# Xinran1205/LBM-Asynchronous

Measured on AMD Instinct MI355X. Metric: MLUPS, higher is better.
Workload: dtype f32

## Files before the change

### include/lbm_hip.h

```cpp
#ifndef LBM_HIP_H
#define LBM_HIP_H

#include <stddef.h>

#ifdef __cplusplus
extern "C" {
#endif

#define LBM_SUCCESS 0
#define LBM_FAILURE 1

#define LBM_ERRORS_DIE    0
#define LBM_ERRORS_RETURN 1

#define LBM_MATH_EXACT 0
#define LBM_MATH_FAST  1

#define LBM_HALO_SYNC  0
#define LBM_HALO_STALE 1
#define LBM_HALO_FRESHEST 2

typedef struct {
  int   nx;
  int   ny;
  int   max_iters;
  int   reynolds_dim;
  float density;
  float accel;
  float omega;
} lbm_params;

typedef struct lbm_ctx lbm_ctx;

typedef struct {
  int    n_slabs;
  int    row_first;
  int    row_count;
  int    fluid_cells;
  int    steps_done;
  int    math_mode;
  int    world_rank;
  int    world_size;
  int    steps_per_launch;
  int    halo_mode;
  int    band_rows;
  int    lane_cells;
  int    nontemporal;
  int    graph_steps;
  int    resident_steps;
  int    resident_min_steps;
  int    resident_rows;
  int    resident_group;
  int    resident_one_xcd;
} lbm_info;

void        lbm_set_error_mode(int mode);
const char* lbm_last_error(void);

const char* lbm_version(void);
int         lbm_device_count(void);

int lbm_partition_rows(int ny, int parts, int index, int* first, int* count);

typedef struct {
  int is_send;
  int peer;
  int row_first;
  int row_count;
} lbm_halo_op;
int lbm_halo_plan(int rows, int parts, int index, int depth, lbm_halo_op out[4]);
int lbm_plan_halo_depth(const lbm_params* params, int parts, int math_mode);

lbm_ctx* lbm_create(const lbm_params* params, const int* obstacles, const float* cells_aos,
                    int n_gpus, int math_mode);

#define LBM_RCCL_ID_BYTES 128
int      lbm_rccl_unique_id(void* id_out);

typedef struct {
  int  loaded;
  int  version;
  int  n_comms;
  int  nranks;
  int  rank;
  char library[512];
} lbm_rccl_status;
// ... 75 lines not shown
```

### lbm-asynchronous_amd/__init__.py

```python
from __future__ import annotations

import ctypes
import os
import subprocess
from dataclasses import dataclass

import numpy as np

_HERE = os.path.dirname(os.path.abspath(__file__))
LIB_PATH = os.environ.get("LBM_LIB") or os.path.join(_HERE, "liblbm_hip.so")
CLI_PATH = os.path.join(_HERE, "d2q9-bgk")

MATH_EXACT = 0
MATH_FAST = 1
_MATH = {"exact": MATH_EXACT, "fast": MATH_FAST, MATH_EXACT: MATH_EXACT, MATH_FAST: MATH_FAST}
RCCL_ID_BYTES = 128
MASK_HALO_ROWS = 3
HALO_SYNC = 0
HALO_STALE = 1
HALO_FRESHEST = 2
_HALO = {"sync": HALO_SYNC, "stale": HALO_STALE, "freshest": HALO_FRESHEST,
         HALO_SYNC: HALO_SYNC, HALO_STALE: HALO_STALE, HALO_FRESHEST: HALO_FRESHEST}

ABI_SYMBOLS = (
    "lbm_set_error_mode", "lbm_last_error", "lbm_version", "lbm_device_count",
    "lbm_partition_rows", "lbm_halo_plan", "lbm_plan_halo_depth", "lbm_create", "lbm_rccl_unique_id", "lbm_rccl_info", "lbm_create_rank", "lbm_create_rank_rows",
    "lbm_create_tiled", "lbm_create_rank_tiled", "lbm_create_rank_hosted", "lbm_create_rank_hosted_rows",
    "lbm_create_rank_hosted_tiled", "lbm_destroy",
    "lbm_get_info", "lbm_set_halo_mode", "lbm_read_halo_log", "lbm_run", "lbm_sync", "lbm_run_timed", "lbm_read_av_vels", "lbm_read_cells",
    "lbm_read_final_state", "lbm_av_velocity", "lbm_total_density", "lbm_calc_reynolds",
    "lbm_set_frames", "lbm_read_frames",
    "lbm_create_batch", "lbm_batch_member", "lbm_batch_run", "lbm_batch_sync", "lbm_batch_get_info", "lbm_destroy_batch",
)


class LbmError(RuntimeError):
    pass


class _CParams(ctypes.Structure):
    _fields_ = [("nx", ctypes.c_int), ("ny", ctypes.c_int), ("max_iters", ctypes.c_int),
                ("reynolds_dim", ctypes.c_int), ("density", ctypes.c_float),
                ("accel", ctypes.c_float), ("omega", ctypes.c_float)]


class _CInfo(ctypes.Structure):
    _fields_ = [("n_slabs", ctypes.c_int), ("row_first", ctypes.c_int), ("row_count", ctypes.c_int),
                ("fluid_cells", ctypes.c_int), ("steps_done", ctypes.c_int),
                ("math_mode", ctypes.c_int), ("world_rank", ctypes.c_int),
                ("world_size", ctypes.c_int), ("steps_per_launch", ctypes.c_int),
                ("halo_mode", ctypes.c_int), ("band_rows", ctypes.c_int), ("lane_cells", ctypes.c_int),
                ("nontemporal", ctypes.c_int), ("graph_steps", ctypes.c_int),
                ("resident_steps", ctypes.c_int), ("resident_min_steps", ctypes.c_int),
                ("resident_rows", ctypes.c_int), ("resident_group", ctypes.c_int), ("resident_one_xcd", ctypes.c_int)]


class _CBatchInfo(ctypes.Structure):
    _fields_ = [("members", ctypes.c_int), ("members_per_launch", ctypes.c_int), ("launches_per_chunk", ctypes.c_int),
                ("resident_steps", ctypes.c_int), ("resident_min_steps", ctypes.c_int), ("steps_done", ctypes.c_int)]


class _CRcclStatus(ctypes.Structure):
    _fields_ = [("loaded", ctypes.c_int), ("version", ctypes.c_int), ("n_comms", ctypes.c_int),
                ("nranks", ctypes.c_int), ("rank", ctypes.c_int), ("library", ctypes.c_char * 512)]


class _CHaloOp(ctypes.Structure):
    _fields_ = [("is_send", ctypes.c_int), ("peer", ctypes.c_int), ("row_first", ctypes.c_int),
                ("row_count", ctypes.c_int)]


_EXCHANGE_FN = ctypes.CFUNCTYPE(ctypes.c_int, ctypes.c_void_p, ctypes.c_int, ctypes.POINTER(_CHaloOp),
                                ctypes.POINTER(ctypes.POINTER(ctypes.c_float)), ctypes.c_size_t)
_ALLREDUCE_FN = ctypes.CFUNCTYPE(ctypes.c_int, ctypes.c_void_p, ctypes.POINTER(ctypes.c_double), ctypes.c_int)


class _CHostComm(ctypes.Structure):
    _fields_ = [("exchange", _EXCHANGE_FN), ("allreduce_sum", _ALLREDUCE_FN), ("user", ctypes.c_void_p)]


@dataclass
class Params:
    nx: int
    ny: int
    max_iters: int
    reynolds_dim: int
    density: float
# ... 530 lines not shown
```

### lbm-asynchronous_amd/csrc/lbm_hip.hip

```cpp
#include "../../include/lbm_hip.h"
#include "lbm_kernels.hip.h"

#include <hip/hip_runtime.h>
#include <hip/hip_ext.h>
#include <rccl/rccl.h>

#include <dlfcn.h>
#include <algorithm>

#include <atomic>
#include <condition_variable>
#include <cstdarg>
#include <cstdio>
#include <cstdlib>
#include <cstring>
#include <functional>
#include <mutex>
#include <thread>
#include <vector>

namespace {

constexpr int kMaxSlabs = 8;
constexpr int kPartSlots = lbm::kPartSlotsMax;
// ... 78 lines not shown
  }
  bool ok = true;
  auto sym = [&](const char* name) -> void* {
    void* p = dlsym(r.handle, name);
    if (!p) { ok = false; snprintf(g_rccl_error, sizeof(g_rccl_error), "librccl lacks %s", name); }
    return p;
  };
#define LBM_RCCL_SYM(field, name) r.field = reinterpret_cast<decltype(r.field)>(sym(name))
  LBM_RCCL_SYM(GetVersion, "ncclGetVersion");        LBM_RCCL_SYM(GetUniqueId, "ncclGetUniqueId");
  LBM_RCCL_SYM(CommInitRank, "ncclCommInitRank");    LBM_RCCL_SYM(CommInitAll, "ncclCommInitAll");
  LBM_RCCL_SYM(CommDestroy, "ncclCommDestroy");      LBM_RCCL_SYM(CommCount, "ncclCommCount");
  LBM_RCCL_SYM(CommUserRank, "ncclCommUserRank");    LBM_RCCL_SYM(GroupStart, "ncclGroupStart");
  LBM_RCCL_SYM(GroupEnd, "ncclGroupEnd");            LBM_RCCL_SYM(Send, "ncclSend");
  LBM_RCCL_SYM(Recv, "ncclRecv");                    LBM_RCCL_SYM(AllReduce, "ncclAllReduce");
  LBM_RCCL_SYM(GetErrorString, "ncclGetErrorString");
#undef LBM_RCCL_SYM
  if (!ok) { r.handle = nullptr; return; }
  Dl_info di;
  if (dladdr(reinterpret_cast<void*>(r.GetVersion), &di) && di.dli_fname) {
    char real[512];
    const char* shown = realpath(di.dli_fname, real) ? real : di.dli_fname;
    strncpy(r.path, shown, sizeof(r.path) - 1);
  }
}

RcclApi* rccl() {
  std::call_once(g_rccl_once, rccl_bind);
  return g_rccl.handle ? &g_rccl : nullptr;
}

#define RCCL_OR_FAIL(ret)                                                       \
  RcclApi* rc_api_ = rccl();                                                    \
  if (!rc_api_) LBM_FAIL(ret, "RCCL is not available: %s", g_rccl_error)

struct Slab {
  int device = 0;
  int row_first = 0;
  int rows = 0;
  int accel_row = lbm::kNoRow;
  int accel_row2 = lbm::kNoRow;
  float* lat_alloc[2] = {nullptr, nullptr};
  float* lat[2] = {nullptr, nullptr};
  unsigned char* mask_alloc = nullptr;
  unsigned char* mask = nullptr;
  float* partials = nullptr;
  double* tot_u = nullptr;
  double* scratch = nullptr;
  double* reduce_buf = nullptr;
  int* flushed_dev = nullptr;
  uint4* res_gran = nullptr;
  float* res_part = nullptr;
  int* res_status = nullptr;
  int* res_status_host = nullptr;
  float* frames = nullptr;
  hipGraphExec_t chunk_graph[2] = {nullptr, nullptr};
  hipStream_t compute = nullptr, comm = nullptr;
  hipEvent_t ev_boundary = nullptr, ev_halo = nullptr, ev_t0 = nullptr, ev_t1 = nullptr;
  hipEvent_t ev_interior[2] = {nullptr, nullptr};
  hipEvent_t ev_flush = nullptr;
  hipEvent_t ev_step = nullptr;
  hipEvent_t ev_fork = nullptr;
  hipEvent_t ev_x[2] = {nullptr, nullptr};
  float* fresh_stage = nullptr;
  unsigned* fresh_arrived = nullptr;
  unsigned* fresh_id_src = nullptr;
  int* fresh_decision = nullptr;
  unsigned char* fresh_log = nullptr;
  hipEvent_t ev_fresh[2] = {nullptr, nullptr};
  ncclComm_t nccl = nullptr;
  lbm::SlotCounts slot_counts;
  int blocks_main = 0;
  int blocks_boundary = 0;
  long fluid_cells = 0;
};

constexpr int kSumBlocks = 1024;
constexpr int kResidentChunk = 4096;
struct TileShape { int tw, th, kmax, threads; void (*exact)(const lbm::TileArgs); void (*fast)(const lbm::TileArgs); };
#define LBM_TILE_SHAPE(TW, TH, K, T) {TW, TH, K, T, lbm::step_tile<0, TW, TH, K, T>, lbm::step_tile<1, TW, TH, K, T>}
const TileShape kTileShapes[] = {
    LBM_TILE_SHAPE(16, 8, 4, 384),
    LBM_TILE_SHAPE(16, 8, 8, 768),
    LBM_TILE_SHAPE(32, 16, 2, 640),
    LBM_TILE_SHAPE(32, 16, 3, 768),
    LBM_TILE_SHAPE(32, 16, 4, 896),
    LBM_TILE_SHAPE(64, 16, 2, 640),
    LBM_TILE_SHAPE(64, 8, 2, 704),
};
constexpr int kTileShapeCount = (int)(sizeof(kTileShapes) / sizeof(kTileShapes[0]));
constexpr int kHaloRows = 4;
constexpr int kMaskHalo = LBM_MASK_HALO_ROWS;
static_assert(kMaskHalo == kHaloRows - 1, "mask halo");

enum ObstacleKind { OBST_GLOBAL = 0, OBST_ROWS = 1, OBST_TILE = 2 };
struct ObstacleSource {
// ... 95 lines not shown
  long plane_stride = 0;
  long row_pitch = 0;
  int n_slabs = 0;
  Slab slab[kMaxSlabs];
  int cur = 0;
  int steps_done = 0;
  int capacity = 0;
  int fluid_cells = 0;
  int math_mode = LBM_MATH_EXACT;
  int halo = HALO_SELF;
  int halo_mode = LBM_HALO_SYNC;
  int rank = 0, world = 1;
  bool ranked = false;
  bool hosted = false;
  lbm_host_comm host_comm = {nullptr, nullptr, nullptr};
  float* host_send[2] = {nullptr, nullptr};
  float* host_recv[2] = {nullptr, nullptr};
  int row_first = 0, row_count = 0;
  int slot_fill = 0;
  long part_stride = 0;
  bool vec4 = false;
  int neigh = 0;
  int nts = 1;
  int snake = 0;
  int fuse2 = 0;
  int pass_steps = 2;
  int prefetch = 0;
  int xcd_chunk = 0;
  int use_stepk = 0;
  int packed = 0;
  int halo_lanes = 1;
  int lds_windows = 0;
  int band_rows = 8, n_strips = 0;
  int lane_cells = 4;
  SlabTeam* team = nullptr;
  int use_graph = 0;
  GraphBuilder* builder = nullptr;
  int resident = 0;
  int resident_min_steps = 16;
  int resident_bands = 0;
  int resident_joint = 0;
  int resident_rows = 4;
  int resident_group = 1;
  int resident_one_xcd = 0;
  long long resident_timeout = 0;
  bool resident_used = false;
  int tile_steps = 0;
  int tile_shape = 0;
  lbm_batch* batch = nullptr;
  int frame_every = 0;
  int frame_slots = 0;
  int frame_ord0 = 0;
  long long frames_written = 0;
  long long frames_read = 0;
};

struct lbm_batch {
  std::vector<lbm_ctx*> members;
  hipStream_t stream = nullptr;
  int resident = 0;
  int member_wgs = 0;
  int members_per_launch = 1;
  int launches = 0;
  int cur = 0;
  int steps_done = 0;
  lbm::ResidentMember* table = nullptr;
// ... 443 lines not shown
        return LBM_SUCCESS;
      }) != LBM_SUCCESS)
    return LBM_FAILURE;
  if (halo &&
      for_slabs(c, [&](int s) -> int {
        Slab& sl = c->slab[s];
        HIP_TRY(LBM_FAILURE, hipSetDevice(sl.device));
        if (q_wait(c, sl.comm, sl.ev_interior[(m + 1) & 1]) != LBM_SUCCESS) return LBM_FAILURE;
        if (c->halo == HALO_MEMCPY) {
          const int north = (s + 1) % c->n_slabs, south = (s - 1 + c->n_slabs) % c->n_slabs;
          if (q_wait(c, sl.comm, c->slab[north].ev_halo) != LBM_SUCCESS) return LBM_FAILURE;
          if (q_wait(c, sl.comm, c->slab[south].ev_halo) != LBM_SUCCESS) return LBM_FAILURE;
        }
        hipEvent_t bdone = bound_events ? sl.ev_boundary : nullptr;
        if (k) {
          const int off = c->n_strips * ceil_div(sl.rows - 2 * k, c->band_rows);
          if (launch_pass(c, s, sl.comm, k, 0, sl.rows, k, sl.rows - k, 2, off, accel_after, bdone) != LBM_SUCCESS) return LBM_FAILURE;
        } else {
          if (launch_step(c, s, sl.comm, 0, sl.rows - 1, 2, sl.blocks_main, accel_after, bdone) != LBM_SUCCESS) return LBM_FAILURE;
        }
        if (!bdone) return q_record(c, sl.ev_boundary, sl.comm);
        return LBM_SUCCESS;
      }) != LBM_SUCCESS)
    return LBM_FAILURE;
  for (int s = 0; s < c->n_slabs; s++) {
    Slab& sl = c->slab[s];
    const int fused_waves = halo ? c->n_strips * (ceil_div(sl.rows - 2 * k, c->band_rows) + 2)
                                 : c->n_strips * ceil_div(sl.rows, c->band_rows);
    const int n_part = tile ? tile_count(c) : (k ? fused_waves : sl.blocks_main + sl.blocks_boundary);
    for (int j = 0; j < adv; j++) sl.slot_counts.n[c->slot_fill + j] = n_part;
  }
  c->cur ^= 1;
  c->slot_fill += adv;
  return LBM_SUCCESS;
}

int chunk_passes(const lbm_ctx* c, int* steps_per_pass) {
  const int halo = (c->halo != HALO_SELF);
  const int adv = (!halo && c->tile_steps) ? c->tile_steps : (c->fuse2 ? c->pass_steps : 1);
  int passes = kPartSlots / adv;
  const int cap = env_int("LBM_GRAPH_PASSES", 0);
  if (cap > 0 && passes > cap) passes = cap;
  passes -= passes & 1;
  *steps_per_pass = adv;
  return passes;
}

bool graph_is_sound(hipGraph_t graph, const char* dump_path) {
  size_t n_nodes = 0, n_edges = 0;
  if (hipGraphGetNodes(graph, nullptr, &n_nodes) != hipSuccess || hipGraphGetEdges(graph, nullptr, nullptr, &n_edges) != hipSuccess)
    return true;
  if (dump_path) fprintf(stderr, "lbm_hip graph: %zu nodes, %zu edges reported\n", n_nodes, n_edges);
  std::vector<hipGraphNode_t> nodes(n_nodes), from(n_edges), to(n_edges);
  if (n_nodes && hipGraphGetNodes(graph, nodes.data(), &n_nodes) != hipSuccess) return true;
  if (n_edges && hipGraphGetEdges(graph, from.data(), to.data(), &n_edges) != hipSuccess) return true;
  auto index_of = [&](hipGraphNode_t x) -> long {
    for (size_t i = 0; i < n_nodes; i++) if (nodes[i] == x) return (long)i;
    return -1;
  };
  std::vector<long> a(n_edges), b(n_edges);
  std::vector<int> indeg(n_nodes, 0);
  size_t self_edges = 0, dup_edges = 0, foreign = 0;
  for (size_t e = 0; e < n_edges; e++) {
    a[e] = index_of(from[e]);
    b[e] = index_of(to[e]);
    if (a[e] < 0 || b[e] < 0) { foreign++; continue; }
// ... 324 lines not shown
                             sl.lat[c->cur], sl.mask, c->plane_stride, c->row_pitch, c->pitch, c->p.nx,
                             sl.accel_row, a1, a2);
          HIP_TRY(LBM_FAILURE, hipGetLastError());
        }
        if (record_t0) HIP_TRY(LBM_FAILURE, hipEventRecord(sl.ev_t0, sl.compute));
        return LBM_SUCCESS;
      }) != LBM_SUCCESS)
    return LBM_FAILURE;

  if (resident) {
    const long long frames = frames_between(c, c->steps_done, (long long)c->steps_done + n_steps);
    if (run_resident(c, n_steps) != LBM_SUCCESS) return LBM_FAILURE;
    c->steps_done += n_steps;
    c->frames_written += frames;
    return LBM_SUCCESS;
  }

  int flushed_upto = c->steps_done;
  int t_first = 0;
  if (c->use_graph) {
    if (replay_chunks(c, n_steps, flushed_upto, &t_first) != LBM_SUCCESS) return LBM_FAILURE;
    flushed_upto += t_first;
  }
  if (halo && reset_pipeline(c) != LBM_SUCCESS) return LBM_FAILURE;

  static const int ext_events = env_int("LBM_EXT_EVENTS", 1);
  const int slots_per_pass = c->tile_steps > c->pass_steps ? c->tile_steps : c->pass_steps;
  int m = 0;
  for (int t = t_first; t < n_steps; m++) {
    const int tile = (!halo && c->tile_steps) ? (c->tile_steps < n_steps - t ? c->tile_steps : n_steps - t) : 0;
    const int k = (!tile && c->fuse2 && n_steps - t >= 2) ? (n_steps - t >= c->pass_steps ? c->pass_steps : 2) : 0;
    const int adv = tile ? tile : (k ? k : 1);
    const bool last = (t + adv == n_steps);
    if (issue_pass(c, m, tile, k, !last, ext_events != 0) != LBM_SUCCESS) return LBM_FAILURE;
    t += adv;
    if (c->slot_fill + slots_per_pass > kPartSlots || last) {
      if (flush_partials(c, flushed_upto) != LBM_SUCCESS) return LBM_FAILURE;
      flushed_upto += c->slot_fill;
      c->slot_fill = 0;
    }
  }
  c->steps_done += n_steps;
  return LBM_SUCCESS;
}

int run_steps(lbm_ctx* c, int n_steps, float* kernel_ms) {
  if (!c) LBM_FAIL(LBM_FAILURE, "lbm_run: null context");
  if (n_steps < 0) LBM_FAIL(LBM_FAILURE, "lbm_run: negative step count");
  if (kernel_ms) *kernel_ms = 0.f;
  if (n_steps == 0) return LBM_SUCCESS;
  if (c->steps_done + n_steps > c->capacity)
    LBM_FAIL(LBM_FAILURE, "lbm_run: %d steps requested but the av_vels record holds %d (maxIters)",
             c->steps_done + n_steps, c->capacity);
  if (frames_fit(c, n_steps, "lbm_run") != LBM_SUCCESS) return LBM_FAILURE;
  if (c->halo != HALO_SELF && c->halo_mode != LBM_HALO_SYNC) return run_steps_stale(c, n_steps, kernel_ms);

  const bool resident = c->resident && n_steps >= c->resident_min_steps;
  if (c->frame_every > 0 && !resident) {
    const int e = c->frame_every;
    for (int t = 0; t < n_steps;) {
      const int tt = c->steps_done, r = tt % e;
      const long long frame_tt = r ? (long long)tt + (e - r) : tt;
      const int seg = (frame_tt - tt + 1 < n_steps - t) ? (int)(frame_tt - tt + 1) : n_steps - t;
      if (run_passes(c, seg, false, kernel_ms && t == 0) != LBM_SUCCESS) return LBM_FAILURE;
      if (c->steps_done - 1 == frame_tt && take_frame(c) != LBM_SUCCESS) return LBM_FAILURE;
      t += seg;
    }
  } else if (run_passes(c, n_steps, resident, kernel_ms != nullptr) != LBM_SUCCESS) {
    return LBM_FAILURE;
// ... 193 lines not shown

void free_slab(Slab& sl) {
  if (hipSetDevice(sl.device) != hipSuccess) return;
  for (int i = 0; i < 2; i++)
    if (sl.chunk_graph[i]) { (void)hipGraphExecDestroy(sl.chunk_graph[i]); sl.chunk_graph[i] = nullptr; }
  if (sl.nccl && g_rccl.CommDestroy) g_rccl.CommDestroy(sl.nccl);
  for (int i = 0; i < 2; i++) if (sl.lat_alloc[i]) (void)hipFree(sl.lat_alloc[i]);
  if (sl.mask_alloc) (void)hipFree(sl.mask_alloc);
  if (sl.partials) (void)hipFree(sl.partials);
  if (sl.tot_u) (void)hipFree(sl.tot_u);
  if (sl.scratch) (void)hipFree(sl.scratch);
  if (sl.reduce_buf) (void)hipFree(sl.reduce_buf);
  if (sl.flushed_dev) (void)hipFree(sl.flushed_dev);
  if (sl.fresh_stage) (void)hipFree(sl.fresh_stage);
  if (sl.fresh_arrived) (void)hipFree(sl.fresh_arrived);
  if (sl.fresh_id_src) (void)hipFree(sl.fresh_id_src);
  if (sl.fresh_decision) (void)hipFree(sl.fresh_decision);
  if (sl.fresh_log) (void)hipFree(sl.fresh_log);
  for (int i = 0; i < 2; i++) if (sl.ev_fresh[i]) (void)hipEventDestroy(sl.ev_fresh[i]);
  if (sl.res_gran) (void)hipFree(sl.res_gran);
  if (sl.res_part) (void)hipFree(sl.res_part);
  if (sl.res_status) (void)hipFree(sl.res_status);
  if (sl.res_status_host) (void)hipHostFree(sl.res_status_host);
  if (sl.frames) (void)hipFree(sl.frames);
  if (sl.ev_boundary) (void)hipEventDestroy(sl.ev_boundary);
  if (sl.ev_halo) (void)hipEventDestroy(sl.ev_halo);
  for (int i = 0; i < 2; i++) if (sl.ev_interior[i]) (void)hipEventDestroy(sl.ev_interior[i]);
  if (sl.ev_flush) (void)hipEventDestroy(sl.ev_flush);
  if (sl.ev_step) (void)hipEventDestroy(sl.ev_step);
  if (sl.ev_fork) (void)hipEventDestroy(sl.ev_fork);
  for (int i = 0; i < 2; i++) if (sl.ev_x[i]) (void)hipEventDestroy(sl.ev_x[i]);
  if (sl.ev_t0) (void)hipEventDestroy(sl.ev_t0);
  if (sl.ev_t1) (void)hipEventDestroy(sl.ev_t1);
  if (sl.compute) (void)hipStreamDestroy(sl.compute);
  if (sl.comm) (void)hipStreamDestroy(sl.comm);
  sl = Slab();
}

bool validate_params(const lbm_params* p) {
  return p && p->nx >= 1 && p->ny >= 2 && p->max_iters >= 0 && (long)p->nx * (long)p->ny <= 2147483647L;
}

struct DeviceTemp {
  void* p = nullptr;
  ~DeviceTemp() { if (p) (void)hipFree(p); }
  template <typename T> T* as() const { return static_cast<T*>(p); }
};

int build_slab(lbm_ctx* c, int s, const ObstacleSource& obst, const float* cells_aos) {
  Slab& sl = c->slab[s];
  const lbm_params& p = c->p;
  HIP_TRY(LBM_FAILURE, hipSetDevice(sl.device));
  HIP_TRY(LBM_FAILURE, hipStreamCreateWithFlags(&sl.compute, hipStreamNonBlocking));
  HIP_TRY(LBM_FAILURE, hipStreamCreateWithFlags(&sl.comm, hipStreamNonBlocking));
  HIP_TRY(LBM_FAILURE, hipEventCreateWithFlags(&sl.ev_boundary, hipEventDisableTiming));
  HIP_TRY(LBM_FAILURE, hipEventCreateWithFlags(&sl.ev_halo, hipEventDisableTiming));
  for (int i = 0; i < 2; i++) HIP_TRY(LBM_FAILURE, hipEventCreateWithFlags(&sl.ev_interior[i], hipEventDisableTiming));
  HIP_TRY(LBM_FAILURE, hipEventCreateWithFlags(&sl.ev_flush, hipEventDisableTiming));
  HIP_TRY(LBM_FAILURE, hipEventCreateWithFlags(&sl.ev_step, hipEventDisableTiming));
  HIP_TRY(LBM_FAILURE, hipEventCreateWithFlags(&sl.ev_fork, hipEventDisableTiming));
  for (int i = 0; i < 2; i++) HIP_TRY(LBM_FAILURE, hipEventCreateWithFlags(&sl.ev_x[i], hipEventDisableTiming));
  HIP_TRY(LBM_FAILURE, hipEventRecord(sl.ev_halo, sl.comm));
  HIP_TRY(LBM_FAILURE, hipEventCreate(&sl.ev_t0));
  HIP_TRY(LBM_FAILURE, hipEventCreate(&sl.ev_t1));

  const size_t lat_bytes = (size_t)(sl.rows + 2 * kHaloRows) * c->row_pitch * sizeof(float);
  for (int i = 0; i < 2; i++) {
    HIP_TRY(LBM_FAILURE, hipMalloc(&sl.lat_alloc[i], lat_bytes));
    HIP_TRY(LBM_FAILURE, hipMemsetAsync(sl.lat_alloc[i], 0, lat_bytes, sl.compute));
    sl.lat[i] = sl.lat_alloc[i] + (size_t)kHaloRows * c->row_pitch;
  }
  HIP_TRY(LBM_FAILURE, hipMalloc(&sl.partials, (size_t)kPartSlots * c->part_stride * sizeof(float)));
  HIP_TRY(LBM_FAILURE, hipMemsetAsync(sl.partials, 0, (size_t)kPartSlots * c->part_stride * sizeof(float), sl.compute));
  HIP_TRY(LBM_FAILURE, hipMalloc(&sl.tot_u, (size_t)(c->capacity > 0 ? c->capacity : 1) * sizeof(double)));
  HIP_TRY(LBM_FAILURE, hipMemsetAsync(sl.tot_u, 0, (size_t)(c->capacity > 0 ? c->capacity : 1) * sizeof(double), sl.compute));
  HIP_TRY(LBM_FAILURE, hipMalloc(&sl.scratch, 2 * kSumBlocks * sizeof(double)));
  HIP_TRY(LBM_FAILURE, hipMalloc(&sl.flushed_dev, sizeof(int)));
  if (c->resident) {
    const size_t gran_bytes = resident_gran_bytes(c);
    HIP_TRY(LBM_FAILURE, hipMalloc(&sl.res_gran, gran_bytes));
    HIP_TRY(LBM_FAILURE, hipMemsetAsync(sl.res_gran, 0, gran_bytes, sl.compute));
    HIP_TRY(LBM_FAILURE, hipMalloc(&sl.res_part, (size_t)kResidentChunk * c->resident_bands * sizeof(float)));
    HIP_TRY(LBM_FAILURE, hipMalloc(&sl.res_status, sizeof(int)));
    HIP_TRY(LBM_FAILURE, hipMemsetAsync(sl.res_status, 0, sizeof(int), sl.compute));
    HIP_TRY(LBM_FAILURE, hipHostMalloc(&sl.res_status_host, sizeof(int)));
    *sl.res_status_host = 0;
  }
  if (c->ranked) HIP_TRY(LBM_FAILURE, hipMalloc(&sl.reduce_buf, (size_t)(c->capacity > 0 ? c->capacity : 1) * sizeof(double)));

  {
    const int mrows = sl.rows + 2 * kMaskHalo;
    const long mask_cells = (long)mrows * c->pitch;
    HIP_TRY(LBM_FAILURE, hipMalloc(&sl.mask_alloc, (size_t)mask_cells));
    HIP_TRY(LBM_FAILURE, hipMemsetAsync(sl.mask_alloc, 0, (size_t)mask_cells, sl.compute));
    sl.mask = sl.mask_alloc + (size_t)kMaskHalo * c->pitch;
    if (obst.kind == OBST_TILE) {
      const size_t tn = (size_t)obst.tile_nx * obst.tile_ny;
// ... 186 lines not shown
      if (owned || in_halo) {
        if (sl.accel_row == lbm::kNoRow || owned) { if (sl.accel_row != lbm::kNoRow) sl.accel_row2 = sl.accel_row; sl.accel_row = local; }
        else sl.accel_row2 = local;
      }
    }
    if (c->halo == HALO_SELF) {
      sl.blocks_main = blocks_for_rows(c, sl.rows);
      sl.blocks_boundary = 0;
    } else {
      if (sl.rows < 2) {
        raise_error(__LINE__, "lbm_create: a slab needs at least 2 rows");
        delete c;
        return nullptr;
      }
      sl.blocks_main = blocks_for_rows(c, sl.rows - 2);
      sl.blocks_boundary = blocks_for_rows(c, 2);
    }
    if (sl.blocks_main + sl.blocks_boundary > max_blocks) max_blocks = sl.blocks_main + sl.blocks_boundary;
  }
  c->fuse2 = plan.fuse2;
  c->lane_cells = plan.lane_cells;
  c->pass_steps = plan.pass_steps;
  c->halo_lanes = ceil_div(c->pass_steps, c->lane_cells);
  c->n_strips = ceil_div(params->nx / c->lane_cells > 0 ? params->nx / c->lane_cells : 1, 64 - 2 * c->halo_lanes);
  c->packed = env_int("LBM_PACKED", 1) ? 1 : 0;
  c->lds_windows = env_int("LBM_LDS_WINDOWS", (c->packed && c->pass_steps == 4) ? 2 : 0);
  if (c->lds_windows < 0 || c->lds_windows > 2 || !c->packed) c->lds_windows = 0;
  c->prefetch = env_int("LBM_PREFETCH", (c->lane_cells == 4 && (c->pass_steps == 3 || (c->pass_steps == 4 && c->lds_windows == 2))) ? 1 : 0) ? 1 : 0;
  const bool many_rounds = (long)c->n_strips * ceil_div(c->row_count / n_slabs, 24) >= 16L * 1024;
  c->xcd_chunk = env_int("LBM_XCD_CHUNK", (c->pass_steps >= 3 && many_rounds) ? c->n_strips : 0);
  if (c->xcd_chunk < 0 || c->xcd_chunk > c->n_strips) c->xcd_chunk = 0;
  c->use_stepk = env_int("LBM_STEPK", 0) ? 1 : 0;

  {
    int pick = (params->nx <= 7168) ? 5 : (params->nx <= 8192 ? 7 : (params->nx <= 12288 ? 5 : 4));
    const long resident = 256L * 4 * 5;
    const long slab_rows = (n_slabs > 1 || world > 1) ? (c->row_count / n_slabs) - 4 : c->row_count;
    const long rows_eff = slab_rows > 1 ? slab_rows : 1;
    if (c->lane_cells == 2 && (long)c->n_strips * ceil_div(rows_eff, 8) < 5 * resident) {
      const long lo = 3;
      long best_cost = -1;
      for (int k = 1; k <= 4; k++) {
        long b = (rows_eff * c->n_strips + k * resident - 1) / (k * resident);
        if (b < lo) b = lo;
        if (b > 32) b = 32;
        const long rounds = ((long)c->n_strips * ceil_div(rows_eff, b) + resident - 1) / resident;
        const long cost = rounds * (b + 2);
        if (best_cost < 0 || cost < best_cost) { best_cost = cost; pick = (int)b; }
      }
    }
    if (c->lane_cells == 2 && c->pass_steps >= 3) {
      const long interior = (n_slabs > 1 || world > 1 || halo_on) ? rows_eff + 4 - 2 * c->pass_steps : rows_eff;
      long b = ((interior > 1 ? interior : 1) * c->n_strips + 2047) / 2048;
      pick = (int)(b < 3 ? 3 : (b > 64 ? 64 : b));
    }
    if (c->lane_cells == 4 && c->pass_steps >= 3) {
      const long interior = (n_slabs > 1 || world > 1 || halo_on) ? rows_eff + 4 - 2 * c->pass_steps : rows_eff;
      const long r_int = interior > 1 ? interior : 1;
      const int warm = 2 * (c->pass_steps - 1);
      if ((long)c->n_strips * ceil_div(r_int, 24) >= 16L * 1024) {
        pick = 32;
      } else {
        double best = -1.0;
        const int b_max = env_int("LBM_BAND_MAX", 160);
        for (int b = 8; b <= b_max; b++) {
          const long waves = (long)c->n_strips * ceil_div(r_int, b);
          const long full = waves / 2048, rest = waves % 2048;
          double rounds = (double)full + (rest == 0 ? 0.0 : (rest > 1024 ? 1.0 : 0.6));
          if (rounds < 1.0) rounds = 1.0;
          const double cost = rounds * (b + warm);
          if (best < 0.0 || cost < best) { best = cost; pick = b; }
        }
      }
    }
    c->band_rows = env_int("LBM_BAND_ROWS", pick);
  }
  if (c->band_rows < 1) c->band_rows = 1;
  for (int s = 0; s < n_slabs; s++) {
    const int waves = c->n_strips * (ceil_div(c->slab[s].rows, c->band_rows) + 2);
    if (c->fuse2 && waves > max_blocks) max_blocks = waves;
  }
  if (!halo_on) {
    const bool other_kernel_requested = getenv("LBM_FUSE2") || getenv("LBM_VEC4");
    const long cells = (long)params->nx * params->ny;
    const int dflt_shape = (cells <= 200L * 1024) ? 0 : 3;
    const int dflt_steps = (other_kernel_requested || cells >= 300L * 1024) ? 0 : kTileShapes[dflt_shape].kmax;
    c->tile_steps = env_int("LBM_TILE_STEPS", dflt_steps);
    c->tile_shape = env_int("LBM_TILE_SHAPE", getenv("LBM_TILE_STEPS") ? (c->tile_steps > 4 ? 1 : 0) : dflt_shape);
    if (c->tile_shape < 0 || c->tile_shape >= kTileShapeCount) c->tile_shape = 0;
    if (c->tile_steps < 0 || c->tile_steps > kTileShapes[c->tile_shape].kmax) c->tile_steps = kTileShapes[c->tile_shape].kmax;
    if (c->tile_steps && tile_count_for(params, c->tile_shape) > max_blocks) max_blocks = tile_count_for(params, c->tile_shape);
  }
  c->part_stride = round_up(max_blocks, 64);

  if (!halo_on && n_slabs == 1) {
    static const char* const selectors[] = {"LBM_FUSE2", "LBM_VEC4", "LBM_TILE_STEPS", "LBM_TILE_SHAPE", "LBM_LANE_CELLS", "LBM_PASS_STEPS",
                                            "LBM_PACKED", "LBM_BAND_ROWS", "LBM_GRAPH", "LBM_STEPK", "LBM_LDS_WINDOWS", "LBM_PREFETCH",
                                            "LBM_XCD_CHUNK", "LBM_NEIGH", "LBM_SNAKE", "LBM_NTS"};
    bool other_kernel = false;
    for (const char* name : selectors) other_kernel = other_kernel || getenv(name) != nullptr;
    const int nx = params->nx, ny = params->ny;
    int cus = 0;
    const int dev = c->slab[0].device;
    if (hipSetDevice(dev) != hipSuccess || hipDeviceGetAttribute(&cus, hipDeviceAttributeMultiprocessorCount, dev) != hipSuccess) cus = 0;
    int rows = env_int("LBM_RESIDENT_ROWS", 0);
    if (rows != 2 && rows != 4) rows = (ny % 2 == 0 && ny / 2 <= cus && ny >= 4) ? 2 : 4;
    const bool shape_ok = nx % 64 == 0 && nx >= 64 && nx <= 1024 && ny % rows == 0 && ny >= 2 * rows;
    if (shape_ok && env_int("LBM_RESIDENT", other_kernel ? 0 : 1)) {
      int per_cu = 0;
      const int joint = (rows == 4 && nx <= 512 && env_int("LBM_RESIDENT_JOINT", nx <= 256 ? 1 : 0)) ? 1 : 0;
      if (cus > 0 && hipOccupancyMaxActiveBlocksPerMultiprocessor(&per_cu, resident_kernel(nx, rows, joint, false), nx, 0) == hipSuccess &&
          per_cu >= 1 && ny / rows <= cus) {
        c->resident = 1;
        c->resident_rows = rows;
        c->resident_bands = ny / rows;
        c->resident_joint = joint;
        {
          const int waves_per_band = nx / 64, cus_per_xcd = cus / 8;
          int group = 1, one_xcd = 0;
          if (rows == 2 && waves_per_band <= 4) {
            for (int g = 1; g * waves_per_band <= 4 && !one_xcd; g *= 2)
              if (c->resident_bands % g == 0 && c->resident_bands / g <= cus_per_xcd) { group = g; one_xcd = 1; }
          }
          one_xcd = env_int("LBM_RESIDENT_ONE_XCD", one_xcd) ? 1 : 0;
// ... 232 lines not shown
lbm_ctx* lbm_create_rank_hosted_rows(const lbm_params* params, const int* obstacle_rows, const float* cells_rows_aos,
                                     int rank, int world_size, const lbm_host_comm* comm, int device, int math_mode) {
  if (!hosted_args_ok(rank, world_size, comm)) return nullptr;
  const ObstacleSource obst = {OBST_ROWS, obstacle_rows, 0, 0, true};
  return create_common(params, obst, cells_rows_aos, 1, math_mode, rank, world_size, nullptr, device, comm);
}

lbm_ctx* lbm_create_rank_hosted_tiled(const lbm_params* params, const int* tile, int tile_nx, int tile_ny,
                                      int rank, int world_size, const lbm_host_comm* comm, int device, int math_mode) {
  if (!hosted_args_ok(rank, world_size, comm)) return nullptr;
  const ObstacleSource obst = {OBST_TILE, tile, tile_nx, tile_ny, false};
  return create_common(params, obst, nullptr, 1, math_mode, rank, world_size, nullptr, device, comm);
}

lbm_ctx* lbm_create_rank_tiled(const lbm_params* params, const int* tile, int tile_nx, int tile_ny,
                               int rank, int world_size, const void* unique_id, int device, int math_mode) {
  if (!rank_args_ok(rank, world_size, unique_id)) return nullptr;
  const ObstacleSource obst = {OBST_TILE, tile, tile_nx, tile_ny, false};
  return create_common(params, obst, nullptr, 1, math_mode, rank, world_size, unique_id, device);
}

void lbm_destroy(lbm_ctx* c) {
  if (!c || c->batch) return;
  if (c->team) {
    c->team->shutdown();
    delete c->team;
    c->team = nullptr;
  }
  for (int s = 0; s < c->n_slabs; s++) {
    if (c->slab[s].compute) {
      (void)hipSetDevice(c->slab[s].device);
      (void)hipStreamSynchronize(c->slab[s].compute);
      (void)hipStreamSynchronize(c->slab[s].comm);
    }
  }
  for (int s = 0; s < c->n_slabs; s++) free_slab(c->slab[s]);
  for (int i = 0; i < 2; i++) {
    if (c->host_send[i]) (void)hipHostFree(c->host_send[i]);
    if (c->host_recv[i]) (void)hipHostFree(c->host_recv[i]);
  }
  delete c;
}

int lbm_get_info(const lbm_ctx* c, lbm_info* out) {
  if (!c || !out) LBM_FAIL(LBM_FAILURE, "lbm_get_info: NULL argument");
  out->n_slabs = c->n_slabs;
  out->row_first = c->row_first;
  out->row_count = c->row_count;
  out->fluid_cells = c->fluid_cells;
  out->steps_done = c->steps_done;
  out->math_mode = c->math_mode;
  out->world_rank = c->rank;
  out->world_size = c->world;
  const bool stale = (c->halo != HALO_SELF && c->halo_mode != LBM_HALO_SYNC);
  out->steps_per_launch = (c->tile_steps && c->halo == HALO_SELF) ? c->tile_steps : ((c->fuse2 && !stale) ? c->pass_steps : 1);
  out->halo_mode = c->halo_mode;
  const bool stream_kernel = c->fuse2 && !stale && !(c->tile_steps && c->halo == HALO_SELF);
  out->band_rows = stream_kernel ? c->band_rows : 0;
  out->lane_cells = stream_kernel ? c->lane_cells : 0;
  out->nontemporal = c->nts;
  {
    int adv = 1;
    const int passes = chunk_passes(c, &adv);
    out->graph_steps = (c->use_graph && !stale) ? passes * adv : 0;
  }
  out->resident_steps = c->resident ? kResidentChunk : 0;
  out->resident_min_steps = c->resident ? c->resident_min_steps : 0;
  out->resident_rows = c->resident ? c->resident_rows : 0;
  out->resident_group = c->resident ? c->resident_group : 0;
  out->resident_one_xcd = c->resident ? c->resident_one_xcd : 0;
  return LBM_SUCCESS;
}

int lbm_set_halo_mode(lbm_ctx* c, int mode) {
  if (!c) LBM_FAIL(LBM_FAILURE, "lbm_set_halo_mode: null context");
  if (mode != LBM_HALO_SYNC && mode != LBM_HALO_STALE && mode != LBM_HALO_FRESHEST) LBM_FAIL(LBM_FAILURE, "lbm_set_halo_mode: unknown mode %d", mode);
  if (mode == LBM_HALO_FRESHEST && c->halo == HALO_HOST) LBM_FAIL(LBM_FAILURE, "lbm_set_halo_mode: the freshest-available mode is not available with the hosted exchange");
  if (mode != LBM_HALO_SYNC && c->frame_every > 0)
    LBM_FAIL(LBM_FAILURE, "lbm_set_halo_mode: animation frames are armed (lbm_set_frames); the stale and freshest halo modes "
             "cannot record them -- disarm with lbm_set_frames(ctx, 0, 0) first");
  c->halo_mode = mode;
  return LBM_SUCCESS;
}

int lbm_set_frames(lbm_ctx* c, int every, int capacity) {
  if (!c) LBM_FAIL(LBM_FAILURE, "lbm_set_frames: null context");
  if (every < 0) LBM_FAIL(LBM_FAILURE, "lbm_set_frames: negative interval %d", every);
  if (every > 0 && capacity < 1) LBM_FAIL(LBM_FAILURE, "lbm_set_frames: capacity %d, at least one frame slot is needed", capacity);
  if (every > 0 && c->halo_mode != LBM_HALO_SYNC)
    LBM_FAIL(LBM_FAILURE, "lbm_set_frames: the context runs the %s halo mode, where splitting a call at a frame would change "
             "the results (every call starts from freshly exchanged halos); frames need LBM_HALO_SYNC",
             c->halo_mode == LBM_HALO_STALE ? "stale" : "freshest");
  if (every > 0 && c->resident) {
    if (c->resident_rows == 4 && c->slab[0].accel_row % 4 != 2)
      LBM_FAIL(LBM_FAILURE, "lbm_set_frames: the lid row %d is not an interior row of a four-row band", c->slab[0].accel_row);
    int per_cu = 0;
    HIP_TRY(LBM_FAILURE, hipSetDevice(c->slab[0].device));
    HIP_TRY(LBM_FAILURE, hipOccupancyMaxActiveBlocksPerMultiprocessor(
                             &per_cu, resident_kernel(c->p.nx, c->resident_rows, c->resident_joint, true), c->p.nx * c->resident_group, 0));
    if (per_cu < 1) LBM_FAIL(LBM_FAILURE, "lbm_set_frames: the resident kernel's frame form does not fit a CU at this shape");
  }
  for (int s = 0; s < c->n_slabs; s++) {
    HIP_TRY(LBM_FAILURE, hipSetDevice(c->slab[s].device));
// ... 74 lines not shown
      HIP_TRY(LBM_FAILURE, hipMemcpyAsync(out + i * frame_cells + (size_t)(sl.row_first - c->row_first) * c->p.nx,
                                          sl.frames + slot * cells, cells * sizeof(float), hipMemcpyDeviceToHost, sl.compute));
    }
    if (steps) steps[i] = (int)((c->frame_ord0 + ord) * c->frame_every);
  }
  for (int s = 0; s < c->n_slabs; s++) {
    HIP_TRY(LBM_FAILURE, hipSetDevice(c->slab[s].device));
    HIP_TRY(LBM_FAILURE, hipStreamSynchronize(c->slab[s].compute));
  }
  c->frames_read += n;
  *n_read = n;
  return LBM_SUCCESS;
}

static const char kMemberRun[] = "%s: this context is a member of a batch (lbm_create_batch); lbm_batch_run advances all its members";

int lbm_run(lbm_ctx* c, int n_steps) {
  if (c && c->batch) LBM_FAIL(LBM_FAILURE, kMemberRun, "lbm_run");
  return run_steps(c, n_steps, nullptr);
}

int lbm_run_timed(lbm_ctx* c, int n_steps, float* kernel_ms_per_step) {
  if (c && c->batch) LBM_FAIL(LBM_FAILURE, kMemberRun, "lbm_run_timed");
  if (!kernel_ms_per_step) LBM_FAIL(LBM_FAILURE, "lbm_run_timed: NULL output");
  return run_steps(c, n_steps, kernel_ms_per_step);
}

int lbm_sync(lbm_ctx* c) {
  if (!c) LBM_FAIL(LBM_FAILURE, "lbm_sync: null context");
  for (int s = 0; s < c->n_slabs; s++) {
    HIP_TRY(LBM_FAILURE, hipSetDevice(c->slab[s].device));
    HIP_TRY(LBM_FAILURE, hipStreamSynchronize(c->slab[s].compute));
    HIP_TRY(LBM_FAILURE, hipStreamSynchronize(c->slab[s].comm));
  }
  if (c->resident_used) {
    const int status = c->batch ? *c->batch->status_host : *c->slab[0].res_status_host;
    c->resident_used = false;
    if (status != 0)
      LBM_FAIL(LBM_FAILURE, "the resident kernel gave up waiting for a neighbouring band after %.0f ms (status %d): its %d workgroups "
               "were not all running at once -- is another process using the device?  The lattice of this context is no "
               "longer valid; LBM_RESIDENT=0 selects the launch-per-pass kernels, LBM_RESIDENT_TIMEOUT_MS moves the bound",
               (double)c->resident_timeout / 1e5, status, c->resident_bands);
  }
  return LBM_SUCCESS;
}

int lbm_read_halo_log(lbm_ctx* c, unsigned char* out, int n) {
  if (!c || !out) LBM_FAIL(LBM_FAILURE, "lbm_read_halo_log: NULL argument");
  if (n < 0 || n > c->steps_done) LBM_FAIL(LBM_FAILURE, "lbm_read_halo_log: %d steps requested, %d recorded", n, c->steps_done);
  if (n == 0) return LBM_SUCCESS;
  if (lbm_sync(c) != LBM_SUCCESS) return LBM_FAILURE;
  std::vector<unsigned char> part((size_t)n);
  for (int s = 0; s < c->n_slabs; s++) {
    Slab& sl = c->slab[s];
    if (sl.fresh_log) {
      HIP_TRY(LBM_FAILURE, hipSetDevice(sl.device));
      HIP_TRY(LBM_FAILURE, hipMemcpy(part.data(), sl.fresh_log, (size_t)n, hipMemcpyDeviceToHost));
    } else {
      part.assign((size_t)n, 3);
    }
    for (int t = 0; t < n; t++) out[(size_t)t * c->n_slabs + s] = part[(size_t)t];
  }
  return LBM_SUCCESS;
}

int lbm_read_av_vels(lbm_ctx* c, float* out, int n) {
// ... 320 lines not shown
```

Measured before the change: 241,200.

## Split single-slab lattice into band groups pipelined across streams with seam passes

```diff
diff --git a/include/lbm_hip.h b/include/lbm_hip.h
--- a/include/lbm_hip.h
+++ b/include/lbm_hip.h
@@ -52,6 +52,7 @@
   int    resident_rows;
   int    resident_group;
   int    resident_one_xcd;
+  int    band_groups;
 } lbm_info;
 
 void        lbm_set_error_mode(int mode);
diff --git a/lbm-asynchronous_amd/__init__.py b/lbm-asynchronous_amd/__init__.py
--- a/lbm-asynchronous_amd/__init__.py
+++ b/lbm-asynchronous_amd/__init__.py
@@ -52,7 +52,8 @@
                 ("halo_mode", ctypes.c_int), ("band_rows", ctypes.c_int), ("lane_cells", ctypes.c_int),
                 ("nontemporal", ctypes.c_int), ("graph_steps", ctypes.c_int),
                 ("resident_steps", ctypes.c_int), ("resident_min_steps", ctypes.c_int),
-                ("resident_rows", ctypes.c_int), ("resident_group", ctypes.c_int), ("resident_one_xcd", ctypes.c_int)]
+                ("resident_rows", ctypes.c_int), ("resident_group", ctypes.c_int), ("resident_one_xcd", ctypes.c_int),
+                ("band_groups", ctypes.c_int)]
 
 
 class _CBatchInfo(ctypes.Structure):
diff --git a/lbm-asynchronous_amd/csrc/lbm_hip.hip b/lbm-asynchronous_amd/csrc/lbm_hip.hip
--- a/lbm-asynchronous_amd/csrc/lbm_hip.hip
+++ b/lbm-asynchronous_amd/csrc/lbm_hip.hip
@@ -134,6 +134,8 @@
 #define RCCL_OR_FAIL(ret)                                                       \
   RcclApi* rc_api_ = rccl();                                                    \
   if (!rc_api_) LBM_FAIL(ret, "RCCL is not available: %s", g_rccl_error)
+
+constexpr int kMaxBandGroups = 3;
 
 struct Slab {
   int device = 0;
@@ -163,6 +165,9 @@
   hipEvent_t ev_step = nullptr;
   hipEvent_t ev_fork = nullptr;
   hipEvent_t ev_x[2] = {nullptr, nullptr};
+  hipStream_t group_extra[kMaxBandGroups - 1] = {nullptr, nullptr};
+  hipEvent_t ev_gi[2][kMaxBandGroups] = {};
+  hipEvent_t ev_gs[2] = {nullptr, nullptr};
   float* fresh_stage = nullptr;
   unsigned* fresh_arrived = nullptr;
   unsigned* fresh_id_src = nullptr;
@@ -324,6 +329,8 @@
   int halo_lanes = 1;
   int lds_windows = 0;
   int band_rows = 8, n_strips = 0;
+  int band_groups = 1;
+  bool groups_forked = false;
   int lane_cells = 4;
   SlabTeam* team = nullptr;
   int use_graph = 0;
@@ -833,6 +840,73 @@
   }
   c->cur ^= 1;
   c->slot_fill += adv;
+  return LBM_SUCCESS;
+}
+
+hipStream_t group_stream(Slab& sl, int g) { return g == 0 ? sl.compute : sl.group_extra[g - 1]; }
+
+int group_fork(lbm_ctx* c, int m) {
+  Slab& sl = c->slab[0];
+  const int prev = (m - 1) & 1;
+  if (q_record(c, sl.ev_gs[prev], sl.compute) != LBM_SUCCESS) return LBM_FAILURE;
+  for (int g = 0; g < c->band_groups; g++)
+    if (q_record(c, sl.ev_gi[prev][g], sl.compute) != LBM_SUCCESS) return LBM_FAILURE;
+  c->groups_forked = true;
+  return LBM_SUCCESS;
+}
+
+int group_join(lbm_ctx* c, int m) {
+  if (!c->groups_forked) return LBM_SUCCESS;
+  Slab& sl = c->slab[0];
+  if (q_wait(c, sl.compute, sl.ev_gs[m & 1]) != LBM_SUCCESS) return LBM_FAILURE;
+  for (int g = 1; g < c->band_groups; g++)
+    if (q_wait(c, sl.compute, sl.ev_gi[m & 1][g]) != LBM_SUCCESS) return LBM_FAILURE;
+  c->groups_forked = false;
+  return LBM_SUCCESS;
+}
+
+int group_rows(const lbm_ctx* c, int g, int* lo, int* hi) {
+  const int rows = c->slab[0].rows, h = rows / c->band_groups;
+  *lo = g * h;
+  *hi = (g == c->band_groups - 1) ? rows : *lo + h;
+  return h;
+}
+int grouped_waves(const lbm_ctx* c, int k) {
+  int bands = c->band_groups;
+  for (int g = 0; g < c->band_groups; g++) {
+    int lo, hi;
+    group_rows(c, g, &lo, &hi);
+    bands += ceil_div(hi - lo - 2 * k, c->band_rows);
+  }
+  return c->n_strips * bands;
+}
+
+int issue_grouped_pass(lbm_ctx* c, int m, int k, bool accel_after, bool bound_events) {
+  Slab& sl = c->slab[0];
+  const int G = c->band_groups, now = m & 1, prev = now ^ 1;
+  int off = 0, h = 0;
+  for (int g = 0; g < G; g++) {
+    int lo, hi;
+    h = group_rows(c, g, &lo, &hi);
+    const hipStream_t st = group_stream(sl, g);
+    if (q_wait(c, st, sl.ev_gs[prev]) != LBM_SUCCESS) return LBM_FAILURE;
+    const int bands = ceil_div(hi - lo - 2 * k, c->band_rows);
+    hipEvent_t done = bound_events ? sl.ev_gi[now][g] : nullptr;
+    if (launch_pass(c, 0, st, k, lo + k, hi - k, c->band_rows, c->band_rows, bands, off, accel_after, done) != LBM_SUCCESS)
+      return LBM_FAILURE;
+    if (!done && q_record(c, sl.ev_gi[now][g], st) != LBM_SUCCESS) return LBM_FAILURE;
+    off += c->n_strips * bands;
+  }
+  for (int g = 0; g < G; g++)
+    if (q_wait(c, sl.comm, sl.ev_gi[prev][g]) != LBM_SUCCESS) return LBM_FAILURE;
+  hipEvent_t sdone = bound_events ? sl.ev_gs[now] : nullptr;
+  if (launch_pass(c, 0, sl.comm, k, -k, (G - 1) * h + k, 2 * k, h, G, off, accel_after, sdone) != LBM_SUCCESS)
+    return LBM_FAILURE;
+  if (!sdone && q_record(c, sl.ev_gs[now], sl.comm) != LBM_SUCCESS) return LBM_FAILURE;
+  off += c->n_strips * G;
+  for (int j = 0; j < k; j++) sl.slot_counts.n[c->slot_fill + j] = off;
+  c->cur ^= 1;
+  c->slot_fill += k;
   return LBM_SUCCESS;
 }
 
@@ -1223,9 +1297,17 @@
     const int k = (!tile && c->fuse2 && n_steps - t >= 2) ? (n_steps - t >= c->pass_steps ? c->pass_steps : 2) : 0;
     const int adv = tile ? tile : (k ? k : 1);
     const bool last = (t + adv == n_steps);
-    if (issue_pass(c, m, tile, k, !last, ext_events != 0) != LBM_SUCCESS) return LBM_FAILURE;
+    const bool grouped = (c->band_groups > 1 && !halo && !tile && k == c->pass_steps);
+    if (grouped) {
+      if (!c->groups_forked && group_fork(c, m) != LBM_SUCCESS) return LBM_FAILURE;
+      if (issue_grouped_pass(c, m, k, !last, ext_events != 0) != LBM_SUCCESS) return LBM_FAILURE;
+    } else {
+      if (group_join(c, m - 1) != LBM_SUCCESS) return LBM_FAILURE;
+      if (issue_pass(c, m, tile, k, !last, ext_events != 0) != LBM_SUCCESS) return LBM_FAILURE;
+    }
     t += adv;
     if (c->slot_fill + slots_per_pass > kPartSlots || last) {
+      if (grouped && group_join(c, m) != LBM_SUCCESS) return LBM_FAILURE;
       if (flush_partials(c, flushed_upto) != LBM_SUCCESS) return LBM_FAILURE;
       flushed_upto += c->slot_fill;
       c->slot_fill = 0;
@@ -1485,6 +1567,11 @@
   for (int i = 0; i < 2; i++) if (sl.ev_x[i]) (void)hipEventDestroy(sl.ev_x[i]);
   if (sl.ev_t0) (void)hipEventDestroy(sl.ev_t0);
   if (sl.ev_t1) (void)hipEventDestroy(sl.ev_t1);
+  for (int i = 0; i < 2; i++) {
+    if (sl.ev_gs[i]) (void)hipEventDestroy(sl.ev_gs[i]);
+    for (int g = 0; g < kMaxBandGroups; g++) if (sl.ev_gi[i][g]) (void)hipEventDestroy(sl.ev_gi[i][g]);
+  }
+  for (int g = 0; g < kMaxBandGroups - 1; g++) if (sl.group_extra[g]) (void)hipStreamDestroy(sl.group_extra[g]);
   if (sl.compute) (void)hipStreamDestroy(sl.compute);
   if (sl.comm) (void)hipStreamDestroy(sl.comm);
   sl = Slab();
@@ -1516,6 +1603,13 @@
   HIP_TRY(LBM_FAILURE, hipEventRecord(sl.ev_halo, sl.comm));
   HIP_TRY(LBM_FAILURE, hipEventCreate(&sl.ev_t0));
   HIP_TRY(LBM_FAILURE, hipEventCreate(&sl.ev_t1));
+  if (c->band_groups > 1) {
+    for (int g = 0; g < c->band_groups - 1; g++) HIP_TRY(LBM_FAILURE, hipStreamCreateWithFlags(&sl.group_extra[g], hipStreamNonBlocking));
+    for (int i = 0; i < 2; i++) {
+      HIP_TRY(LBM_FAILURE, hipEventCreateWithFlags(&sl.ev_gs[i], hipEventDisableTiming));
+      for (int g = 0; g < c->band_groups; g++) HIP_TRY(LBM_FAILURE, hipEventCreateWithFlags(&sl.ev_gi[i][g], hipEventDisableTiming));
+    }
+  }
 
   const size_t lat_bytes = (size_t)(sl.rows + 2 * kHaloRows) * c->row_pitch * sizeof(float);
   for (int i = 0; i < 2; i++) {
@@ -1768,6 +1862,11 @@
   if (c->xcd_chunk < 0 || c->xcd_chunk > c->n_strips) c->xcd_chunk = 0;
   c->use_stepk = env_int("LBM_STEPK", 0) ? 1 : 0;
 
+  if (!halo_on && n_slabs == 1 && c->fuse2 && !c->use_graph) {
+    c->band_groups = env_int("LBM_BAND_GROUPS", (c->lane_cells == 4 && c->pass_steps == 4) ? 2 : 1);
+    if (c->band_groups < 1) c->band_groups = 1;
+    if (c->band_groups > kMaxBandGroups) c->band_groups = kMaxBandGroups;
+  }
   {
     int pick = (params->nx <= 7168) ? 5 : (params->nx <= 8192 ? 7 : (params->nx <= 12288 ? 5 : 4));
     const long resident = 256L * 4 * 5;
@@ -1791,16 +1890,18 @@
       pick = (int)(b < 3 ? 3 : (b > 64 ? 64 : b));
     }
     if (c->lane_cells == 4 && c->pass_steps >= 3) {
-      const long interior = (n_slabs > 1 || world > 1 || halo_on) ? rows_eff + 4 - 2 * c->pass_steps : rows_eff;
+      const int groups = c->band_groups;
+      const long interior = (n_slabs > 1 || world > 1 || halo_on) ? rows_eff + 4 - 2 * c->pass_steps
+                                                                  : (groups > 1 ? rows_eff / groups - 2 * c->pass_steps : rows_eff);
       const long r_int = interior > 1 ? interior : 1;
       const int warm = 2 * (c->pass_steps - 1);
-      if ((long)c->n_strips * ceil_div(r_int, 24) >= 16L * 1024) {
+      if (groups * (long)c->n_strips * ceil_div(r_int, 24) >= 16L * 1024) {
         pick = 32;
       } else {
         double best = -1.0;
         const int b_max = env_int("LBM_BAND_MAX", 160);
         for (int b = 8; b <= b_max; b++) {
-          const long waves = (long)c->n_strips * ceil_div(r_int, b);
+          const long waves = groups * (long)c->n_strips * ceil_div(r_int, b);
           const long full = waves / 2048, rest = waves % 2048;
           double rounds = (double)full + (rest == 0 ? 0.0 : (rest > 1024 ? 1.0 : 0.6));
           if (rounds < 1.0) rounds = 1.0;
@@ -1812,10 +1913,15 @@
     c->band_rows = env_int("LBM_BAND_ROWS", pick);
   }
   if (c->band_rows < 1) c->band_rows = 1;
+  if (c->band_groups > 1) {
+    const int interior = c->row_count / c->band_groups - 2 * c->pass_steps;
+    if (interior < (getenv("LBM_BAND_GROUPS") ? 1 : 2 * c->band_rows)) c->band_groups = 1;
+  }
   for (int s = 0; s < n_slabs; s++) {
     const int waves = c->n_strips * (ceil_div(c->slab[s].rows, c->band_rows) + 2);
     if (c->fuse2 && waves > max_blocks) max_blocks = waves;
   }
+  if (c->band_groups > 1 && grouped_waves(c, c->pass_steps) > max_blocks) max_blocks = grouped_waves(c, c->pass_steps);
   if (!halo_on) {
     const bool other_kernel_requested = getenv("LBM_FUSE2") || getenv("LBM_VEC4");
     const long cells = (long)params->nx * params->ny;
@@ -1826,6 +1932,7 @@
     if (c->tile_shape < 0 || c->tile_shape >= kTileShapeCount) c->tile_shape = 0;
     if (c->tile_steps < 0 || c->tile_steps > kTileShapes[c->tile_shape].kmax) c->tile_steps = kTileShapes[c->tile_shape].kmax;
     if (c->tile_steps && tile_count_for(params, c->tile_shape) > max_blocks) max_blocks = tile_count_for(params, c->tile_shape);
+    if (c->tile_steps) c->band_groups = 1;
   }
   c->part_stride = round_up(max_blocks, 64);
 
@@ -2124,6 +2231,7 @@
       (void)hipSetDevice(c->slab[s].device);
       (void)hipStreamSynchronize(c->slab[s].compute);
       (void)hipStreamSynchronize(c->slab[s].comm);
+      for (hipStream_t g : c->slab[s].group_extra) if (g) (void)hipStreamSynchronize(g);
     }
   }
   for (int s = 0; s < c->n_slabs; s++) free_slab(c->slab[s]);
@@ -2161,6 +2269,7 @@
   out->resident_rows = c->resident ? c->resident_rows : 0;
   out->resident_group = c->resident ? c->resident_group : 0;
   out->resident_one_xcd = c->resident ? c->resident_one_xcd : 0;
+  out->band_groups = stream_kernel ? c->band_groups : 1;
   return LBM_SUCCESS;
 }
 
@@ -2301,6 +2410,7 @@
     HIP_TRY(LBM_FAILURE, hipSetDevice(c->slab[s].device));
     HIP_TRY(LBM_FAILURE, hipStreamSynchronize(c->slab[s].compute));
     HIP_TRY(LBM_FAILURE, hipStreamSynchronize(c->slab[s].comm));
+    for (hipStream_t g : c->slab[s].group_extra) if (g) HIP_TRY(LBM_FAILURE, hipStreamSynchronize(g));
   }
   if (c->resident_used) {
     const int status = c->batch ? *c->batch->status_host : *c->slab[0].res_status_host;
```

Result: faster. 266,100 (median of 6 runs) (+10.4%).
